# utiasSTARS/pyslam

Hardware: AMD Instinct MI355X
Metric: ms/LM-iter (Jac build + J^T J + Schur solve), stereo BA @ 500k residuals (lower is better)
Workload: dtype f64

## Files before the change

### pyslam_amd/csrc/ps_abi_problem.h

```cpp


const char* ps_last_error(void) { return g_err.c_str(); }

int ps_device_count(void) {
    int n = 0;
    if (hipGetDeviceCount(&n) != hipSuccess) return 0;
    return n;
}

int ps_warm_up(void) {
    static std::once_flag once;
    static int rc = 0;
    std::call_once(once, [] {
        void* p = nullptr;
        if (hipMalloc(&p, 256) != hipSuccess) { rc = fail("hipMalloc failed (no usable HIP device?)"); return; }
        hipLaunchKernelGGL(k_zero4, dim3(1), dim3(256), 0, 0, (size_t)8, (double*)p, (size_t)0, (double*)nullptr, (size_t)0,
                           (double*)nullptr, (size_t)0, (double*)nullptr);
        double hostw[4] = {0, 0, 0, 0};
        (void)hipMemsetAsync(p, 0, 256, 0);
        (void)hipMemcpyAsync((char*)p + 128, p, 64, hipMemcpyDeviceToDevice, 0);
        (void)hipMemcpyAsync(hostw, p, sizeof(hostw), hipMemcpyDeviceToHost, 0);
        if (hipDeviceSynchronize() != hipSuccess) rc = fail("the warm-up launch failed");
        hipFree(p);
        hipFuncAttributes a;
// ... 16 lines not shown
        PS_TOUCH(k_pcg_spmv<6>); PS_TOUCH(k_pcg_spmv<3>); PS_TOUCH(k_ldi_init); PS_TOUCH(k_ldi_update); PS_TOUCH(k_ldi_gemm); PS_TOUCH(k_ldi_mirror);
        PS_TOUCH(k_ldi_ritz); PS_TOUCH(k_ldi_seed_prep); PS_TOUCH(k_ldi_fro_total); PS_TOUCH(k_ldi_pad_identity);
        PS_TOUCH(k_ldi_scaled_dense<6>); PS_TOUCH(k_ldi_sym_unscale<6>); PS_TOUCH(k_ldi_scaled_dense<3>); PS_TOUCH(k_ldi_sym_unscale<3>);
        PS_TOUCH(k_shard_pack<6>); PS_TOUCH(k_shard_unpack<6>); PS_TOUCH(k_publish); PS_TOUCH(k_cov_rhs); PS_TOUCH(k_triangulate<false>);
        PS_TOUCH(k_scale_blocks<3>); PS_TOUCH(k_rows_setup<3, PS_RS_REGS>); PS_TOUCH(k_rows_setup<3, PS_RS_EXACT>); PS_TOUCH(k_coarse_rowsums<3>); PS_TOUCH(k_coarse_matrix<3>);
        PS_TOUCH(k_coarse_chol<3, true>); PS_TOUCH(k_coarse_border<3>); PS_TOUCH(k_coarse_mreduce<3>); PS_TOUCH(k_coarse_xbuild<3>);
        PS_TOUCH(k_coarse_recover<3>); PS_TOUCH(k_cg_fused_lds<3, 8>); PS_TOUCH(k_cg_unscale<3>);
#undef PS_TOUCH
    });
    return rc;
}

int ps_problem_destroy(ps_problem* h) {
    if (!h) return 0;
    if (h->cp_dbg) {
        long long c[8]; hipMemcpy(c, h->cp_dbg, 64, hipMemcpyDeviceToHost);
        int khz = 100000; hipDeviceGetAttribute(&khz, hipDeviceAttributeWallClockRate, 0);
        fprintf(stderr, "k_cg_persist, workgroup 0, %ld launches, us per launch: recurrences %.2f | sync %.2f | products + publish %.2f | gather + sums %.2f "
                "(%.1f failed passes) | dots + sync %.2f | exchanges %lld = %.2f per launch\n", h->cp_launches, c[0] * 1e3 / khz / h->cp_launches,
                c[1] * 1e3 / khz / h->cp_launches, c[2] * 1e3 / khz / h->cp_launches, c[3] * 1e3 / khz / h->cp_launches, (double)c[7] / h->cp_launches,
                c[5] * 1e3 / khz / h->cp_launches, c[6], (double)c[6] / h->cp_launches);
        hipFree(h->cp_dbg);
    }
    if (h->xp_dbg) {
        std::vector<long long> c(3 * 64 * 8); hipMemcpy(c.data(), h->xp_dbg, c.size() * 8, hipMemcpyDeviceToHost);
        int khz = 100000; hipDeviceGetAttribute(&khz, hipDeviceAttributeWallClockRate, 0);
        for (int w = 0; w < 3; ++w) {
            double ph[6] = {0, 0, 0, 0, 0, 0}; int np = 0;
            for (int p = 1; p < 64; ++p) {
                const long long* t = &c[((size_t)w * 64 + p) * 8];
                if (!t[6] || !t[4]) break;
                ph[0] += t[0] - t[6]; ph[1] += t[1] - t[0]; ph[2] += t[2] - t[1]; ph[3] += t[5] - t[2]; ph[4] += t[3] - t[5]; ph[5] += t[4] - t[3]; ++np;
            }
            const double u = 1e3 / khz / std::max(np, 1);
            fprintf(stderr, "k_xcg_persist, workgroup %s, last launch, %d passes, us per pass: t + coarse y %.2f | columns %.2f | products + publish %.2f | "
                    "first gather pass %.2f | rest of the gather %.2f | record sums + dots %.2f | sum %.2f\n", w == 0 ? "0" : (w == 1 ? "nwg/2" : "nwg-1"), np,
// ... 471 lines not shown
```

### pyslam_amd/csrc/ps_abi_solver.h

```cpp

int ps_get_info(ps_problem* h, ps_problem_info* info) {
    if (!h || !info) return fail("null argument");
    info->dof = h->D; info->num_poses = h->P; info->num_reduced = h->nr; info->num_points = h->L;
    info->num_var_points = h->nv; info->num_obs = h->N; info->num_edges = h->F; info->num_priors = 0;
    info->reduced_nnzb = h->nnzb; info->num_pairs = h->npairs;
    info->reduce_count = ((long)h->nnzb + h->nr) / 2 * h->D * h->D + (long)h->nr * h->D + 3;
    info->device_bytes = (int64_t)h->dev_bytes;
    info->cg_restarts = h->cg_fallbacks;
    info->cg_kernel_launches = h->cg_kernel_launches;
    info->ldi_solves = h->ldi_solves; info->ldi_fallbacks = h->ldi_fallbacks; info->ldi_seeds = h->ldi_seeds;
    info->xcg_fused_solves = h->xf_solves; info->xcg_fused_fallbacks = h->xf_fallbacks;
    info->cg_persist_solves = h->cp_launches; info->cg_persist_failures = h->cp_failures;
    info->cg_persist_refused = h->cp_refused; info->persist_cus = h->persist_cus;
    info->persist_cus_needed = h->cp_ok ? h->cp_cus_needed : (h->xp_ok ? h->xp_cus_needed : 0);
    info->landmark_passes_taken_over = h->prelm_used;
    return 0;
}

int ps_eval_cost(ps_problem* h, int include_all_constant, double* cost) {
    if (!h || !cost) return fail("null argument");
    if (include_all_constant && h->fuse_cost == 1 && lm_cost_possible(h)) { if (lm_cost_pass(h, h->lin_lambda, SC_COST)) return -1; }
    else if (cost_pass(h, include_all_constant, SC_COST)) return -1;
    if (read_scalars(h)) return -1;
    *cost = h->h_scalars[SC_COST];
// ... 849 lines not shown
int ps_set_option(ps_problem* h, const char* name, double value) {
    if (!h || !name) return fail("null argument");
    if (!std::strcmp(name, "expect_next")) { h->expect_next = value != 0 && !h->hybrid; return 0; }
    if (!std::strcmp(name, "solve_horizon")) { h->solve_horizon = value < 0 ? -1 : (int)std::min(value, 1e6); return 0; }
    if (!std::strcmp(name, "setup_ride")) {
        h->setup_ride = value != 0 ? 1 : 0;
        h->prelin_valid = h->prelm_valid = false;
        relook_launch_gates(h);
        return 0;
    }
    if (!std::strcmp(name, "rows_regs")) {
        h->rows_regs = value != 0 ? 1 : 0;
        h->prelin_valid = h->prelm_valid = h->ride_valid = false;
        return 0;
    }
    h->prelin_valid = h->prelm_valid = h->ride_valid = false;
    const char* refusal = nullptr;
    const int fx = ps_option_apply(*h, name, value, &refusal);
    if (fx == PS_OPT_UNKNOWN) return fail(std::string("unknown option: ") + name);
    if (fx == PS_OPT_REFUSED) return fail(refusal);
    if (fx & PS_FX_COARSE_REBUILD) h->coarse_built = false;
    if (fx & PS_FX_DROP_FACTOR) h->lci_next = -1;
    if (fx & PS_FX_DROP_SIDE) h->side_todo = false;
    if ((fx & PS_FX_LDI_OFF) && !h->ldi_enable) { h->ldi_cur = -1; if (h->ldi_state != 1) h->ldi_state = 0; }
    if (fx & PS_FX_RELOOK_PATH) relook_path(h);
    relook_launch_gates(h);
    return 0;
}

int ps_get_option(ps_problem* h, const char* name, double* value) {
    if (!h || !name || !value) return fail("null argument");
    const std::string n(name);
    if (n == "lin_zero_list") *value = h->lin_zero_gate ? 1.0 : 0.0;
    else if (n == "lin_fills") *value = (double)h->lin_fills;
    else if (n == "lin_zero_launches") *value = (double)h->lin_zero_launches;
    else if (n == "setup_ride") *value = h->ride_gate ? 1.0 : 0.0;
    else if (n == "factor_launches") *value = (double)h->bjf_launches;
    else if (n == "factors_ridden") *value = (double)h->bjf_ridden;
    else if (n == "factor_plan_mismatches") *value = (double)h->bjf_mismatches;
    else if (n == "rows_regs") *value = (double)h->rows_regs;
    else if (n == "rows_setups") *value = (double)h->rows_setups;
    else if (n == "exact_row_setups") *value = (double)h->exact_row_setups;
    else if (n == "rows_lci_in_lds") *value = h->coarse_built && h->lagx_ok && h->rows_lci_lds ? 1.0 : 0.0;
    else return fail("ps_get_option: no read-back for option: " + n);
    return 0;
}

int ps_reset_solver_state(ps_problem* h) {
    if (!h) return fail("null argument");
    h->prelin_valid = h->prelm_valid = h->ride_valid = false;
    if (!h->solver_touched) {
        static_cast<PsCostHistory&>(*h) = PsCostHistory{};
        return 0;
    }
    h->solver_touched = false;
    HIP_OK(hipStreamSynchronize(h->stream));
    if (h->side) HIP_OK(hipStreamSynchronize(h->side));
    if (h->ldi_stream) HIP_OK(hipStreamSynchronize(h->ldi_stream));
// ... 62 lines not shown
```

### pyslam_amd/csrc/ps_core.hip

```cpp
#include <hip/hip_runtime.h>

#include <algorithm>
#include <array>
#include <map>
#include <atomic>
#include <chrono>
#include <thread>
#include <climits>
#include <cmath>
#include <cstdio>
#include <cstring>
#include <memory>
#include <mutex>
#include <string>
#include <vector>

#include "pyslam_hip.h"
#include "ps_kernels.h"
#include "ps_ransac_core.h"
#include "ps_ransac.h"
#include "ps_k_twoview.h"
#include "ps_k_pnp.h"
#include "ps_k_sim3.h"
#include "ps_photo.h"
// ... 267 lines not shown
    bool xf_one_ok = false, xf_two = false;
    int32_t *xf_cptr = nullptr, *xf_cols = nullptr, *xf_nlo = nullptr, *xf_nhi = nullptr, *xf_rec = nullptr;
    uint16_t* xf_lidx = nullptr;
    double *xf_tq[2] = {}, *xf_ts[2] = {}, *xf_t[2] = {};
    int xf_rmax = 1, xf_nwg = 0, xf_pf = 2;
    size_t xf_nrec = 0;
    long xf_solves = 0, xf_fallbacks = 0;
    bool cp_ok = false;
    bool cp_recovered = false;
    int cp_ntasks = 0, cg_max_launches = 0;
    void* cp_tasks = nullptr;
    int32_t* cp_row_task0 = nullptr;
    unsigned long long* cp_exch = nullptr;
    unsigned cp_salt = 0;
    long cp_launches = 0, cp_failures = 0;
    int persist_dev = 0, persist_cus = 0;
    bool persist_masked = false;
    int cp_cus_needed = 0, xp_cus_needed = 0;
    int persist_held = 0;
    bool params_moved_since_lin = false;
    bool z_foreign = false;
    bool no_repeat = false;
    long cp_refused = 0;
    void persist_release() { if (persist_held) { ps_persist_ledger().release(persist_dev, persist_held); persist_held = 0; } }
    int persist_capacity() const { return persist_masked ? persist_cus / 2 : persist_cus; }
    bool persist_reserve(int need) {
        if (need <= 0 || persist_cus <= 0) return false;
        if (persist_held) return true;
        if (!ps_persist_ledger().reserve(persist_dev, need, persist_capacity())) { ++cp_refused; return false; }
        persist_held = need; return true;
// ... 239 lines not shown
```

### pyslam_amd/csrc/ps_host_cg.h

```cpp

namespace {

struct StageTimer {
    ps_problem* h;
    int stage;
    hipEvent_t a = nullptr, b = nullptr;
    int slot = -1;
    StageTimer(ps_problem* h_, int st, int level = 2) : h(h_), stage(st) {
        if (h->profiling < level) return;
        if (h->profiling == 1 && h->prof_every > 1 &&
            h->prof_tick % h->prof_every != (st == PS_ST_CG_KERNEL ? h->prof_every / 2 : 0)) return;
        if (h->ev_used + 2 > h->ev_pool.size()) {
            for (int i = 0; i < 64; ++i) { hipEvent_t e; hipEventCreate(&e); h->ev_pool.push_back(e); }
        }
        slot = (int)h->ev_used;
        a = h->ev_pool[h->ev_used++];
        b = h->ev_pool[h->ev_used++];
        hipEventRecord(a, h->stream);
    }
    void stop() {
        if (!a) return;
        hipEventRecord(b, h->stream);
        h->pending.push_back({stage, slot});
        a = nullptr;
// ... 311 lines not shown
        h->upload(&h->aug_slot, slot) || h->upload(&h->fine_nnz, fnz)) return -1;
    lap("uploads");
    h->cp_ok = false;
    if (!h->cg_explicit && !split && (long)(nr + ncb) * D <= PS_CP_MAXN) {
        const int rows = nr + ncb;
        std::vector<CpTask> tasks;
        std::vector<int32_t> rt0(rows + 1, 0);
        for (int i = 0; i < rows; ++i) {
            rt0[i] = (int32_t)tasks.size();
            const int w = i < nr ? std::min(arp[i + 1] - arp[i], fnz[i] + ncb) : arp[i + 1] - arp[i];
            const int nt = std::max(1, cdiv(w, PS_CP_TASKB)), per = cdiv(w, nt);
            for (int k = 0; k < nt; ++k) tasks.push_back(CpTask{i, arp[i] + k * per, std::min(arp[i] + w, arp[i] + (k + 1) * per), 0});
        }
        rt0[rows] = (int32_t)tasks.size();
        const int cp_nwg = cdiv((int)tasks.size(), PS_CP_NT / 64);
        int cp_per_cu = 0;
        {
            const void* kfn = D == 6 ? (const void*)k_cg_persist<6> : (const void*)k_cg_persist<3>;
            if (hipOccupancyMaxActiveBlocksPerMultiprocessor(&cp_per_cu, kfn, PS_CP_NT, 0) != hipSuccess) { (void)hipGetLastError(); cp_per_cu = 0; }
        }
        h->cp_cus_needed = cp_per_cu > 0 ? cdiv(cp_nwg, cp_per_cu) : 0;
        if ((long)tasks.size() * D <= (long)PS_CP_MAXEX && h->cp_cus_needed > 0 && h->cp_cus_needed <= h->persist_capacity()) {
            CpTask* dt = nullptr;
            if (h->upload(&dt, tasks) || h->upload(&h->cp_row_task0, rt0) ||
                h->alloc(&h->cp_exch, (size_t)4 * tasks.size() * D)) return -1;
            h->cp_tasks = dt;
            HIP_OK(hipMemsetAsync(h->cp_exch, 0, (size_t)4 * tasks.size() * D * sizeof(unsigned long long), h->stream));
            h->cp_ntasks = (int)tasks.size(); h->cp_salt = 0; h->cp_ok = true;
        }
    }
    if (h->alloc(&h->BSZ, (h->cg_explicit ? eq.size() : (size_t)nr * ncb) * D * D) || h->alloc(&h->Bmat2[0], (size_t)nr * D * D) ||
        h->alloc(&h->bgv, (size_t)nr * D) || h->alloc(&h->SB, (size_t)aci.size() * D * D)) return -1;
    h->Bmat = h->Bmat2[0];
    h->lagx_ok = !h->cg_explicit && !split && h->nc <= 96 && maxlen <= PS_RS_MAXROW;
// ... 371 lines not shown
    return 0;
}

int side_kick(ps_problem* h) {
    if (!h->side_todo) return 0;
    return h->D == 6 ? cg_side_kick<6>(h) : cg_side_kick<3>(h);
}

template <int D>
void cg_fused_launch(ps_problem* h, double tol, int count) {
    const int cap = h->hist_cap;
    const int rows = h->cg_split ? h->nr : h->nr_aug;
    const int ncbs = h->cg_split ? h->ncb : 0;
    const double tol2 = tol * tol;
#ifdef PS_MEASURE
    if (ps_env("PS_CP_CLOCKS") && !h->cp_dbg) { hipMalloc(&h->cp_dbg, 64); hipMemset(h->cp_dbg, 0, 64); }
#endif
    if (h->cg_persist && h->cp_ok && h->G > 0 && h->cg_lds && !h->cg_split && !h->cg_two_level_reduce &&
        !h->cg_ablate && h->cg_launched == 0 && h->cg_max_launches > 0 && h->cg_max_launches <= 4090 && !h->no_repeat &&
        h->persist_reserve(h->cp_cus_needed)) {
        const int nl = h->cg_max_launches;
        if (++h->cp_salt >= (1u << 20)) {
            hipMemsetAsync(h->cp_exch, 0, (size_t)4 * h->cp_ntasks * D * sizeof(unsigned long long), h->stream);
            h->cp_salt = 1;
        }
        hipLaunchKernelGGL((k_cg_persist<D>), dim3(cdiv(h->cp_ntasks, PS_CP_NT / 64)), dim3(PS_CP_NT), 0, h->stream, h->nr_aug * D,
                           h->cp_ntasks, (const CpTask*)h->cp_tasks, h->cp_row_task0, h->acol_idx, h->Saug, h->cg_r[0], h->cg_w[0], h->cg_s[0], h->cg_p,
                           h->cg_xh, h->hist, cap, nl, tol2, h->status, h->scalars, h->cp_exch, h->cp_salt, h->cp_spin, h->cp_dbg,
                           CpRecover{h->nr, h->ncb, h->pnode, h->pw0, h->pw1, h->Linv, h->Lci2[h->lci_cur], h->Bmat, h->x});
        h->cg_launched = nl; h->cg_kernel_launches += 1; ++h->cp_launches;
        h->cp_recovered = true;
        return;
    }
    h->cg_kernel_launches += count;
    for (int i = 0; i < count; ++i, ++h->cg_launched) {
        const int n = h->cg_launched, o = n & 1, nw = o ^ 1;
        const double* tot = h->cg_two_level_reduce ? h->cg_tot : nullptr;
        if (tot && !h->cg_split && n > 0)
            hipLaunchKernelGGL(k_cg_reduce, dim3(1), dim3(1024), 0, h->stream, rows, h->cg_gd[o], h->cg_tot, h->status);
#define PS_CG_LAUNCH(NWV)                                                                                          \
        hipLaunchKernelGGL((k_cg_fused<D, NWV>), dim3(rows), dim3(64 * NWV), 0, h->stream, rows, h->arow_ptr,           \
                           h->acol_idx, h->Saug, h->cg_r[o], h->cg_w[o], h->cg_s[o], h->cg_r[nw], h->cg_w[nw],        \
                           h->cg_s[nw], h->cg_p, h->cg_xh, h->cg_gd[o], h->cg_gd[nw], h->hist, cap, n - 1, tol2,      \
                           h->status, h->scalars, h->nr, h->ell_wf, h->ell_wc, h->cg_ablate, tot, ncbs,              \
                           h->fine_nnz, h->cg_cgd[o], h->cg_U, h->cg_ab)
        if (h->cg_lds && !h->cg_short_rows && !h->cg_split && !tot && !h->cg_ablate && rows <= 1024 &&
// ... 434 lines not shown
```

### pyslam_amd/csrc/ps_k_cg_fused.h

```cpp
#pragma once

template <int D>
__global__ __launch_bounds__(256) void k_block_jacobi_factor(
    int nr, const int32_t* __restrict__ diag_slot, const double* __restrict__ S,
    double* __restrict__ Linv, int32_t* __restrict__ status,
    const double* __restrict__ g, double* __restrict__ r0, double* __restrict__ w0, double* __restrict__ s0,
    double* __restrict__ p0, double* __restrict__ x0,
    const double* __restrict__ poses, const int32_t* __restrict__ pose_of_rid, int basis,
    double* __restrict__ Bmat, double* __restrict__ bg)
{
    constexpr int DD = D * D;
    __shared__ double sc[4][PS_BJF_SCRATCH(D)];
    const int wv = threadIdx.x >> 6, lane = threadIdx.x & 63;
    const int i = blockIdx.x * 4 + wv;
    if (i >= nr) return;
    double a_in = 0.0;
    if (lane < DD) a_in = S[(size_t)diag_slot[i] * DD + lane];
    if (g && lane < D) sc[wv][3 * DD + D + lane] = g[(size_t)i * D + lane];
    const BjFactorOut o{Linv, status, g ? r0 : nullptr, w0, s0, p0, x0, poses, pose_of_rid, basis, Bmat, bg};
    block_jacobi_factor_wave<D>(i, lane, a_in, sc[wv], o);
}

template <int D>
__global__ __launch_bounds__(64) void k_scale_blocks(
// ... 737 lines not shown
    int nr, const int32_t* __restrict__ row_ptr, const int32_t* __restrict__ col_idx, const double* __restrict__ S,
    const double* __restrict__ x, const double* __restrict__ gsaved, double* __restrict__ g)
{
    const int t = blockIdx.x * blockDim.x + threadIdx.x;
    if (t >= nr * D) return;
    const int i = t / D, r = t % D;
    double v = gsaved[t];
    for (int b = row_ptr[i]; b < row_ptr[i + 1]; ++b) {
        const double* sb = S + (size_t)b * D * D + r * D;
        const double* xv = x + (size_t)col_idx[b] * D;
#pragma unroll
        for (int c = 0; c < D; ++c) v -= sb[c] * xv[c];
    }
    g[t] = v;
}
```

### pyslam_amd/csrc/ps_k_cg_persist.h

```cpp
#pragma once

#define PS_CP_NT 512
#define PS_CP_NQ 6
#define PS_CP_TASKB (8 * PS_CP_NQ)
#define PS_CP_NV 4
#define PS_CP_MAXEX (12 * PS_CP_NT)
#define PS_CP_MAXN (PS_CP_NV * PS_CP_NT)
#define PS_CP_LONG 4
#define PS_PERSIST_TIMEOUT_TICKS 100000000LL
#ifndef PS_CP_SLEEP
#define PS_CP_SLEEP 1
#endif

struct CpTask { int32_t row, b0, b1, pad; };
struct CpRecover { int nr, ncb; const int32_t* pnode; const double *pw0, *pw1, *Linv, *Lci, *Bmat; double* x; };

typedef unsigned long long ps_u64;
typedef __attribute__((address_space(1))) ps_u64 ps_gu64;

typedef unsigned ps_u32x4 __attribute__((ext_vector_type(4)));
PS_DEV void cp_put(ps_u64* g, unsigned tag, double v) {
    const ps_u64 b = (ps_u64)__double_as_longlong(v);
    const ps_u32x4 q = {(unsigned)(b & 0xffffffffull), tag, (unsigned)(b >> 32), tag};
    asm volatile("global_store_dwordx4 %0, %1, off sc1\n\ts_nop 1" :: "v"(g), "v"(q) : "memory");
}

PS_DEV ps_u64 cp_get(const ps_u64* buf, unsigned off) {
    return __hip_atomic_load((const ps_gu64*)((const char*)buf + off), __ATOMIC_RELAXED, __HIP_MEMORY_SCOPE_AGENT);
}

template <int D>
__global__ __launch_bounds__(PS_CP_NT) void k_cg_persist(
    int n , int ntasks, const CpTask* __restrict__ tasks,
    const int32_t* __restrict__ row_task0 ,
    const int32_t* __restrict__ acol_idx, const double* __restrict__ Saug,
    const double* __restrict__ r0, const double* __restrict__ w0, const double* __restrict__ s0,
    double* __restrict__ p_io, double* __restrict__ x_io,
    double* __restrict__ hist, int cap, int nlaunch , double tol2,
    int32_t* __restrict__ status, double* __restrict__ scalars,
    ps_u64* __restrict__ exch , unsigned salt, unsigned spin_limit,
    long long* __restrict__ dbg , CpRecover rec)
{
    constexpr int DD = D * D;
    __shared__ double rn[PS_CP_MAXN];
    __shared__ double yc[PS_CP_MAXN];
    __shared__ double red[2][2][PS_CP_NT / 64];
    __shared__ int bad;
    const int t = threadIdx.x, wv = t >> 6, lane = t & 63, kk = lane >> 3, r = lane & 7;
    const int task = blockIdx.x * (PS_CP_NT / 64) + wv;
    const bool chief = blockIdx.x == 0 && t == 0;
    const size_t nex = (size_t)ntasks * D;
    if (t == 0) bad = 0;
    int b0 = 0, b1 = 0;
    if (task < ntasks) { const CpTask tk = tasks[task]; b0 = tk.b0; b1 = tk.b1; }
    int cj[PS_CP_NQ];
    double sv[PS_CP_NQ][D];
#pragma unroll
    for (int q = 0; q < PS_CP_NQ; ++q) {
        const int b = b0 + kk + 8 * q;
        cj[q] = 0;
#pragma unroll
        for (int c = 0; c < D; ++c) sv[q][c] = 0.0;
        if (b < b1 && r < D) {
            cj[q] = acol_idx[b] * D;
            const double* sb = Saug + (size_t)b * DD + r * D;
#pragma unroll
            for (int c = 0; c < D; ++c) sv[q][c] = sb[c];
// ... 2 lines not shown
    double vr[PS_CP_NV], vw[PS_CP_NV], vs[PS_CP_NV], vp[PS_CP_NV], vx[PS_CP_NV];
    int e0[PS_CP_NV], en[PS_CP_NV];
#pragma unroll
    for (int v = 0; v < PS_CP_NV; ++v) {
        const int i = t + v * PS_CP_NT;
        vr[v] = vw[v] = vs[v] = vp[v] = vx[v] = 0.0; e0[v] = 0; en[v] = 0;
        if (i < n) {
            vr[v] = r0[i]; vw[v] = w0[i]; vs[v] = s0[i]; vp[v] = p_io[i]; vx[v] = x_io[i];
            const int row = i / D, ta = row_task0[row];
            e0[v] = ta * D + (i - row * D); en[v] = row_task0[row + 1] - ta;
        }
    }
    int lv = -1, le0 = 0, len = 0;
#pragma unroll
    for (int v = PS_CP_NV - 1; v >= 0; --v) if (en[v] > 2) { lv = v; le0 = e0[v]; len = en[v]; }
    if (status[ST_PCG_DONE]) return;
    double gamma = 0.0, delta = 0.0, inv_gprev = 0.0, inv_aprev = 0.0, thresh = 0.0;
    bool converged = false;
    long long ck[8] = {0, 0, 0, 0, 0, 0, 0, 0};
#define PS_CP_CLK(i) do { if (dbg) { const long long now_ = wall_clock64(); ck[i] += now_ - last_; last_ = now_; } } while (0)
    long long last_ = dbg ? wall_clock64() : 0;
    for (int k = -1; k < nlaunch - 1; ++k) {
        double alpha = 0.0, beta = 0.0;
        if (k >= 0) {
            if (k == 0) thresh = tol2 * gamma;
            if (!(gamma > thresh)) {
                if (chief) { status[ST_PCG_DONE] = (gamma != gamma) ? 2 : 1; scalars[SC_RRFINAL] = gamma; if (k == 0) scalars[SC_RR0] = gamma; }
                converged = !(gamma != gamma);
                break;
            }
            beta = (k == 0) ? 0.0 : gamma * inv_gprev;
            const double denom = (k == 0) ? delta : delta - beta * gamma * inv_aprev;
            alpha = gamma / denom;
            if (!(denom > 0.0)) {
                if (chief) { status[ST_PCG_DONE] = 2; scalars[SC_RRFINAL] = gamma; }
                break;
            }
            if (chief) {
                hist[k] = gamma; hist[cap + k] = alpha; status[ST_PCG_ITERS] = k + 1; scalars[SC_RRFINAL] = gamma;
                if (k == 0) { scalars[SC_THRESH] = thresh; scalars[SC_RR0] = gamma; }
            }
        }
        const double gamma_now = gamma, alpha_now = alpha;
        double gs = 0.0;
#pragma unroll
        for (int v = 0; v < PS_CP_NV; ++v) {
            const int i = t + v * PS_CP_NT;
            const double sn = vw[v] + beta * vs[v];
            const double pn = vr[v] + beta * vp[v];
            const double rnv = cg_rnew(vr[v], vw[v], vs[v], alpha, beta);
            vs[v] = sn; vp[v] = pn; vx[v] += alpha * pn; vr[v] = rnv;
            if (i < n) { rn[i] = rnv; gs += rnv * rnv; }
        }
        double (*rd)[PS_CP_NT / 64] = red[k & 1];
        gs = wave_sum(gs);
        if (lane == 0) rd[0][wv] = gs;
        PS_CP_CLK(0);
        __syncthreads();
        PS_CP_CLK(1);
        double gamma_next = 0.0;
#pragma unroll
        for (int w2 = 0; w2 < PS_CP_NT / 64; ++w2) gamma_next += rd[0][w2];
        if (k >= 0 && k + 1 < nlaunch - 1 && !(gamma_next > thresh)) {
            if (chief) { status[ST_PCG_DONE] = (gamma_next != gamma_next) ? 2 : 1; scalars[SC_RRFINAL] = gamma_next; }
            converged = !(gamma_next != gamma_next);
            break;
        }
        const unsigned tag = salt * 4096u + (unsigned)(k + 2);
        ps_u64* buf = exch + (size_t)(k & 1) * nex * 2;
        {
            double acc = 0.0;
#pragma unroll
            for (int q = 0; q < PS_CP_NQ; ++q) {
                const double* v = rn + cj[q];
#pragma unroll
                for (int c = 0; c < D; ++c) acc += sv[q][c] * v[c];
            }
            acc += __shfl_xor(acc, 8, 64);
            acc += __shfl_xor(acc, 16, 64);
// ... 63 lines not shown
                    if (spins > spin_limit || (long long)wall_clock64() - t_enter > PS_PERSIST_TIMEOUT_TICKS) { bad = 1; break; }
                    if (PS_CP_SLEEP) __builtin_amdgcn_s_sleep(PS_CP_SLEEP);
                    ck[7] += 1;
                }
            }
        }
        PS_CP_CLK(3);
        double ds = 0.0;
#pragma unroll
        for (int v = 0; v < PS_CP_NV; ++v) ds += vw[v] * vr[v];
        ds = wave_sum(ds);
        if (lane == 0) rd[1][wv] = ds;
        __syncthreads();
        PS_CP_CLK(5);
        if (bad) {
            if (t == 0) { status[ST_PCG_DONE] = 2; status[ST_PERSIST_FAIL] = 1; }
            break;
        }
        gamma = gamma_next; delta = 0.0;
#pragma unroll
        for (int w2 = 0; w2 < PS_CP_NT / 64; ++w2) delta += rd[1][w2];
    }
    if (dbg && chief) for (int i = 0; i < 8; ++i) dbg[i] += ck[i];
#undef PS_CP_CLK
    if (blockIdx.x == 0) {
        if (converged && rec.x) {
            const int nc = rec.ncb * D, nf = rec.nr * D;
            __syncthreads();
#pragma unroll
            for (int v = 0; v < PS_CP_NV; ++v) { const int i = t + v * PS_CP_NT; if (i < n) rn[i] = vx[v]; }
            __syncthreads();
            const double* xc = rn + nf;
            for (int base = 0; base < nc; base += PS_CP_NT / 8) {
                const int kq = base + t / 8, sub = t & 7;
                double v = 0.0;
                if (kq < nc) for (int m = kq + sub; m < nc; m += 8) v += rec.Lci[(size_t)m * nc + kq] * xc[m];
                v += __shfl_xor(v, 1, 64); v += __shfl_xor(v, 2, 64); v += __shfl_xor(v, 4, 64);
                if (kq < nc && sub == 0) yc[kq] = v;
            }
            __syncthreads();
            for (int e = t; e < nf; e += PS_CP_NT) {
                const int i = e / D, c = e - i * D, q = rec.pnode[i];
                const double w0 = rec.pw0[i], w1 = rec.pw1[i];
                double z[D];
#pragma unroll
                for (int m = 0; m < D; ++m) z[m] = w0 * yc[q * D + m] + ((q + 1 < rec.ncb) ? w1 * yc[(q + 1) * D + m] : 0.0);
                double v = 0.0;
#pragma unroll
                for (int a = 0; a < D; ++a) {
                    double xhat = rn[i * D + a];
#pragma unroll
                    for (int m = 0; m < D; ++m) xhat += rec.Bmat[(size_t)i * DD + a * D + m] * z[m];
                    v += rec.Linv[(size_t)i * DD + a * D + c] * xhat;
                }
                rec.x[e] = v;
            }
        }
#pragma unroll
        for (int v = 0; v < PS_CP_NV; ++v) {
            const int i = t + v * PS_CP_NT;
            if (i < n) { x_io[i] = vx[v]; p_io[i] = vp[v]; }
        }
    }
}
```

### pyslam_amd/csrc/ps_k_coarse.h

```cpp
#pragma once


PS_DEV double coarse_weight(int j, int q, const int32_t* __restrict__ pnode,
                            const double* __restrict__ pw0, const double* __restrict__ pw1) {
    return (pnode[j] == q) ? pw0[j] : pw1[j];
}

template <int D>
__global__ __launch_bounds__(256) void k_coarse_rowsums(
    int nr, int ncb, const int32_t* __restrict__ run_lo, const int32_t* __restrict__ run_hi,
    const int32_t* __restrict__ acol_idx, const int32_t* __restrict__ pnode,
    const double* __restrict__ pw0, const double* __restrict__ pw1,
    const double* __restrict__ SB ,
    double* __restrict__ SZ, const double* __restrict__ Bmat, double* __restrict__ BSZ )
{
    constexpr int DD = D * D;
    extern __shared__ double srow[];
    const int i = blockIdx.x, nslot = ncb * DD;
    double* sBi = srow + nslot;
    if (threadIdx.x < DD) sBi[threadIdx.x] = Bmat[(size_t)i * DD + threadIdx.x];
    for (int t = threadIdx.x; t < nslot; t += blockDim.x) {
        const int q = t / DD, e = t % DD;
        const int k0 = run_lo[i * ncb + q], k1 = run_hi[i * ncb + q];
        double acc = 0.0;
// ... 587 lines not shown

template <int D>
__global__ __launch_bounds__(256) void k_coarse_recover(
    int nr, int ncb, const int32_t* __restrict__ pnode, const double* __restrict__ pw0,
    const double* __restrict__ pw1, const double* __restrict__ Linv, const double* __restrict__ Lci,
    const double* __restrict__ xh, double* __restrict__ x, const int32_t* __restrict__ gate,
    const double* __restrict__ Bmat)
{
    __shared__ double sy[400];
    if (gate && gate[ST_PCG_DONE] != 1) return;
    const int nc = ncb * D;
    const double* xc = xh + (size_t)nr * D;
    for (int base = 0; base < nc; base += blockDim.x / 8) {
        const int k = base + threadIdx.x / 8, sub = threadIdx.x & 7;
        double v = 0.0;
        if (k < nc) {
#pragma unroll 4
            for (int m = k + sub; m < nc; m += 8) v += Lci[(size_t)m * nc + k] * xc[m];
        }
        v += __shfl_xor(v, 1, 64); v += __shfl_xor(v, 2, 64); v += __shfl_xor(v, 4, 64);
        if (k < nc && sub == 0) sy[k] = v;
    }
    __syncthreads();
    const int t = blockIdx.x * blockDim.x + threadIdx.x;
    if (t >= nr * D) return;
    const int i = t / D, c = t % D, q = pnode[i];
    const double w0 = pw0[i], w1 = pw1[i];
    double z[D];
#pragma unroll
    for (int m = 0; m < D; ++m) z[m] = w0 * sy[q * D + m] + ((q + 1 < ncb) ? w1 * sy[(q + 1) * D + m] : 0.0);
    double v = 0.0;
#pragma unroll
    for (int a = 0; a < D; ++a) {
        double xhat = xh[(size_t)i * D + a];
#pragma unroll
        for (int m = 0; m < D; ++m) xhat += Bmat[(size_t)i * D * D + a * D + m] * z[m];
        v += Linv[(size_t)i * D * D + a * D + c] * xhat;
    }
    x[t] = v;
}

#define PS_RS_THREADS 1024
#define PS_RS_MAXROW 96
#define PS_RS_WAVES 0
#define PS_RS_REGS 1
#define PS_RS_EXACT 2

template <int D, int MODE>
__global__ __launch_bounds__(PS_RS_THREADS) void k_rows_setup(
    int nr, int ncb, const int32_t* __restrict__ row_ptr, const int32_t* __restrict__ col_idx,
    const int32_t* __restrict__ aug_slot, const double* __restrict__ S, const double* __restrict__ Linv,
    const double* __restrict__ Blag, const double* __restrict__ Bcur,
    const int32_t* __restrict__ arow_ptr, const int32_t* __restrict__ fine_nnz,
    const int32_t* __restrict__ run_lo, const int32_t* __restrict__ run_hi,
// ... 232 lines not shown
```

### pyslam_amd/device.py

```python
import ctypes as C

import numpy as np

from pyslam_amd import _native as nat


COVARIANCE_MARGINALS_LIMIT = 12288


def _solve_options(o, opt, linesearch=None):
    o.max_iters, o.allow_nondecreasing_steps = int(opt.max_iters), int(bool(opt.allow_nondecreasing_steps))
    o.max_nondecreasing_steps = int(opt.max_nondecreasing_steps)
    o.linesearch = int(bool(opt.linesearch_max_iters > 0 if linesearch is None else linesearch))
    o.min_update_norm, o.min_cost = float(opt.min_update_norm), float(opt.min_cost)
    o.min_cost_decrease, o.lm_lambda = float(opt.min_cost_decrease), float(getattr(opt, 'lm_lambda', 0.))
    return o


class DeviceProblem:
    def __init__(self, lp, stream=None, extra_pairs=None):
        lib = nat.require_gpu()
        self._lib = lib
        self.lp = lp
        self.dof = lp.dof
# ... 383 lines not shown
    def cg_restarts(self):
        info = nat.ProblemInfo()
        nat.check(self._lib.ps_get_info(self._h, C.byref(info)))
        return int(info.cg_restarts)

    def cg_kernel_launches(self):
        info = nat.ProblemInfo()
        nat.check(self._lib.ps_get_info(self._h, C.byref(info)))
        return int(info.cg_kernel_launches)

    def cg_persist_counts(self):
        info = nat.ProblemInfo()
        nat.check(self._lib.ps_get_info(self._h, C.byref(info)))
        return int(info.cg_persist_solves), int(info.cg_persist_failures)

    def set_option(self, name, value):
        nat.check(self._lib.ps_set_option(self._h, name.encode(), float(value)))

    def get_option(self, name):
        v = C.c_double()
        nat.check(self._lib.ps_get_option(self._h, name.encode(), C.byref(v)))
        return v.value

    def set_profiling(self, level=2):
        nat.check(self._lib.ps_set_profiling(self._h, int(level)))

    def stage_times(self, reset=False):
        ms = (C.c_double * nat.PS_NUM_STAGES)()
        cnt = (C.c_int64 * nat.PS_NUM_STAGES)()
        nat.check(self._lib.ps_get_stage_times(self._h, ms, cnt, int(reset)))
# ... 314 lines not shown
```

Measured before the change: 0.2809.

## Distribute coarse solution recovery across all persistent CG workgroups with LDS prefetch

```diff
diff --git a/pyslam_amd/csrc/ps_abi_problem.h b/pyslam_amd/csrc/ps_abi_problem.h
--- a/pyslam_amd/csrc/ps_abi_problem.h
+++ b/pyslam_amd/csrc/ps_abi_problem.h
@@ -54,12 +54,12 @@
 int ps_problem_destroy(ps_problem* h) {
     if (!h) return 0;
     if (h->cp_dbg) {
-        long long c[8]; hipMemcpy(c, h->cp_dbg, 64, hipMemcpyDeviceToHost);
+        long long c[PS_CP_NCLK]; hipMemcpy(c, h->cp_dbg, sizeof c, hipMemcpyDeviceToHost);
         int khz = 100000; hipDeviceGetAttribute(&khz, hipDeviceAttributeWallClockRate, 0);
         fprintf(stderr, "k_cg_persist, workgroup 0, %ld launches, us per launch: recurrences %.2f | sync %.2f | products + publish %.2f | gather + sums %.2f "
-                "(%.1f failed passes) | dots + sync %.2f | exchanges %lld = %.2f per launch\n", h->cp_launches, c[0] * 1e3 / khz / h->cp_launches,
+                "(%.1f failed passes) | dots + sync %.2f | exchanges %lld = %.2f per launch | prologue %.2f | recovery %.2f\n", h->cp_launches, c[0] * 1e3 / khz / h->cp_launches,
                 c[1] * 1e3 / khz / h->cp_launches, c[2] * 1e3 / khz / h->cp_launches, c[3] * 1e3 / khz / h->cp_launches, (double)c[7] / h->cp_launches,
-                c[5] * 1e3 / khz / h->cp_launches, c[6], (double)c[6] / h->cp_launches);
+                c[5] * 1e3 / khz / h->cp_launches, c[6], (double)c[6] / h->cp_launches, c[8] * 1e3 / khz / h->cp_launches, c[4] * 1e3 / khz / h->cp_launches);
         hipFree(h->cp_dbg);
     }
     if (h->xp_dbg) {
diff --git a/pyslam_amd/csrc/ps_abi_solver.h b/pyslam_amd/csrc/ps_abi_solver.h
--- a/pyslam_amd/csrc/ps_abi_solver.h
+++ b/pyslam_amd/csrc/ps_abi_solver.h
@@ -887,6 +887,17 @@
         h->prelin_valid = h->prelm_valid = h->ride_valid = false;
         return 0;
     }
+    if (!std::strcmp(name, "cg_persist_recover")) {
+        h->cg_persist_recover = value != 0 ? 1 : 0;
+        h->prelin_valid = h->prelm_valid = h->ride_valid = false;
+        return 0;
+    }
+    if (!std::strcmp(name, "cg_persist_recover_lds")) {
+        if (!(value >= 0 && value <= PS_CP_RECOVER_LDS_CAP)) return fail("cg_persist_recover_lds out of range (0 .. 146432 bytes)");
+        h->cg_persist_recover_lds = (int)value;
+        h->prelin_valid = h->prelm_valid = h->ride_valid = false;
+        return 0;
+    }
     h->prelin_valid = h->prelm_valid = h->ride_valid = false;
     const char* refusal = nullptr;
     const int fx = ps_option_apply(*h, name, value, &refusal);
@@ -915,6 +926,11 @@
     else if (n == "rows_setups") *value = (double)h->rows_setups;
     else if (n == "exact_row_setups") *value = (double)h->exact_row_setups;
     else if (n == "rows_lci_in_lds") *value = h->coarse_built && h->lagx_ok && h->rows_lci_lds ? 1.0 : 0.0;
+    else if (n == "cg_persist_recover") *value = (double)h->cg_persist_recover;
+    else if (n == "cg_persist_recover_lds") *value = (double)h->cg_persist_recover_lds;
+    else if (n == "cg_persist_recover_need") *value = h->coarse_built && h->cp_ok ? (double)h->cp_rec_lds : 0.0;
+    else if (n == "cg_persist_recovered") *value = (double)h->cp_rec_inside;
+    else if (n == "cg_persist_recover_fallbacks") *value = (double)h->cp_rec_behind;
     else return fail("ps_get_option: no read-back for option: " + n);
     return 0;
 }
diff --git a/pyslam_amd/csrc/ps_core.hip b/pyslam_amd/csrc/ps_core.hip
--- a/pyslam_amd/csrc/ps_core.hip
+++ b/pyslam_amd/csrc/ps_core.hip
@@ -305,6 +305,11 @@
     unsigned long long* cp_exch = nullptr;
     unsigned cp_salt = 0;
     long cp_launches = 0, cp_failures = 0;
+    int cg_persist_recover = 1;
+    int cg_persist_recover_lds = PS_CP_RECOVER_LDS_CAP;
+    int cp_rec_pp = 0, cp_rec_cols = 0;
+    size_t cp_rec_lds = 0;
+    long cp_rec_inside = 0, cp_rec_behind = 0;
     int persist_dev = 0, persist_cus = 0;
     bool persist_masked = false;
     int cp_cus_needed = 0, xp_cus_needed = 0;
diff --git a/pyslam_amd/csrc/ps_host_cg.h b/pyslam_amd/csrc/ps_host_cg.h
--- a/pyslam_amd/csrc/ps_host_cg.h
+++ b/pyslam_amd/csrc/ps_host_cg.h
@@ -349,10 +349,22 @@
         }
         rt0[rows] = (int32_t)tasks.size();
         const int cp_nwg = cdiv((int)tasks.size(), PS_CP_NT / 64);
+        h->cp_rec_pp = cdiv(nr, cp_nwg); h->cp_rec_cols = 0; h->cp_rec_lds = 0;
+        {
+            bool ascending = true;
+            for (int i = 1; i < nr; ++i) ascending = ascending && pnode[i] >= pnode[i - 1];
+            for (int p0 = 0; p0 < nr && ascending; p0 += h->cp_rec_pp) {
+                const int last = std::min(nr, p0 + h->cp_rec_pp) - 1;
+                h->cp_rec_cols = std::max(h->cp_rec_cols, (std::min(ncb - 1, pnode[last] + 1) - pnode[p0] + 1) * D);
+            }
+            if (ascending && h->cp_rec_pp <= PS_CP_NT) h->cp_rec_lds = cp_recover_lds(D, ncb * D, h->cp_rec_pp, h->cp_rec_cols);
+        }
         int cp_per_cu = 0;
         {
             const void* kfn = D == 6 ? (const void*)k_cg_persist<6> : (const void*)k_cg_persist<3>;
-            if (hipOccupancyMaxActiveBlocksPerMultiprocessor(&cp_per_cu, kfn, PS_CP_NT, 0) != hipSuccess) { (void)hipGetLastError(); cp_per_cu = 0; }
+            const size_t dyn = h->cp_rec_lds <= (size_t)PS_CP_RECOVER_LDS_CAP ? h->cp_rec_lds : 0;
+            if (dyn && ensure_dynamic_lds(kfn, dyn)) return -1;
+            if (hipOccupancyMaxActiveBlocksPerMultiprocessor(&cp_per_cu, kfn, PS_CP_NT, dyn) != hipSuccess) { (void)hipGetLastError(); cp_per_cu = 0; }
         }
         h->cp_cus_needed = cp_per_cu > 0 ? cdiv(cp_nwg, cp_per_cu) : 0;
         if ((long)tasks.size() * D <= (long)PS_CP_MAXEX && h->cp_cus_needed > 0 && h->cp_cus_needed <= h->persist_capacity()) {
@@ -754,7 +766,7 @@
     const int ncbs = h->cg_split ? h->ncb : 0;
     const double tol2 = tol * tol;
 #ifdef PS_MEASURE
-    if (ps_env("PS_CP_CLOCKS") && !h->cp_dbg) { hipMalloc(&h->cp_dbg, 64); hipMemset(h->cp_dbg, 0, 64); }
+    if (ps_env("PS_CP_CLOCKS") && !h->cp_dbg) { hipMalloc(&h->cp_dbg, PS_CP_NCLK * 8); hipMemset(h->cp_dbg, 0, PS_CP_NCLK * 8); }
 #endif
     if (h->cg_persist && h->cp_ok && h->G > 0 && h->cg_lds && !h->cg_split && !h->cg_two_level_reduce &&
         !h->cg_ablate && h->cg_launched == 0 && h->cg_max_launches > 0 && h->cg_max_launches <= 4090 && !h->no_repeat &&
@@ -764,12 +776,15 @@
             hipMemsetAsync(h->cp_exch, 0, (size_t)4 * h->cp_ntasks * D * sizeof(unsigned long long), h->stream);
             h->cp_salt = 1;
         }
-        hipLaunchKernelGGL((k_cg_persist<D>), dim3(cdiv(h->cp_ntasks, PS_CP_NT / 64)), dim3(PS_CP_NT), 0, h->stream, h->nr_aug * D,
+        const bool inside = h->cg_persist_recover && h->cp_rec_lds > 0 && h->cp_rec_lds <= (size_t)h->cg_persist_recover_lds;
+        hipLaunchKernelGGL((k_cg_persist<D>), dim3(cdiv(h->cp_ntasks, PS_CP_NT / 64)), dim3(PS_CP_NT), inside ? h->cp_rec_lds : 0, h->stream, h->nr_aug * D,
                            h->cp_ntasks, (const CpTask*)h->cp_tasks, h->cp_row_task0, h->acol_idx, h->Saug, h->cg_r[0], h->cg_w[0], h->cg_s[0], h->cg_p,
                            h->cg_xh, h->hist, cap, nl, tol2, h->status, h->scalars, h->cp_exch, h->cp_salt, h->cp_spin, h->cp_dbg,
-                           CpRecover{h->nr, h->ncb, h->pnode, h->pw0, h->pw1, h->Linv, h->Lci2[h->lci_cur], h->Bmat, h->x});
+                           CpRecover{h->nr, h->ncb, h->pnode, h->pw0, h->pw1, h->Linv, h->Lci2[h->lci_cur], h->Bmat, inside ? h->x : nullptr,
+                                     h->cp_rec_pp, h->cp_rec_cols});
         h->cg_launched = nl; h->cg_kernel_launches += 1; ++h->cp_launches;
-        h->cp_recovered = true;
+        ++(inside ? h->cp_rec_inside : h->cp_rec_behind);
+        h->cp_recovered = inside;
         return;
     }
     h->cg_kernel_launches += count;
diff --git a/pyslam_amd/csrc/ps_k_cg_fused.h b/pyslam_amd/csrc/ps_k_cg_fused.h
--- a/pyslam_amd/csrc/ps_k_cg_fused.h
+++ b/pyslam_amd/csrc/ps_k_cg_fused.h
@@ -775,3 +775,26 @@
     }
     g[t] = v;
 }
+
+PS_DEV double coarse_recover_ylane(const double* col, int stride, const double* xc, int k, int sub, int nc) {
+    double v = 0.0;
+#pragma unroll 4
+    for (int m = k + sub; m < nc; m += 8) v = fma(col[(size_t)m * stride], xc[m], v);
+    return v;
+}
+template <int D>
+PS_DEV double coarse_recover_entry(const double* y0, const double* y1, double w0, double w1, const double* xh ,
+                                   const double* B , const double* Li , int c) {
+    double z[D];
+#pragma unroll
+    for (int m = 0; m < D; ++m) { const double right = y1 ? w1 * y1[m] : 0.0; z[m] = fma(w0, y0[m], right); }
+    double v = 0.0;
+#pragma unroll
+    for (int a = 0; a < D; ++a) {
+        double xhat = xh[a];
+#pragma unroll
+        for (int m = 0; m < D; ++m) xhat = fma(B[a * D + m], z[m], xhat);
+        v = fma(Li[a * D + c], xhat, v);
+    }
+    return v;
+}
diff --git a/pyslam_amd/csrc/ps_k_cg_persist.h b/pyslam_amd/csrc/ps_k_cg_persist.h
--- a/pyslam_amd/csrc/ps_k_cg_persist.h
+++ b/pyslam_amd/csrc/ps_k_cg_persist.h
@@ -7,13 +7,18 @@
 #define PS_CP_MAXEX (12 * PS_CP_NT)
 #define PS_CP_MAXN (PS_CP_NV * PS_CP_NT)
 #define PS_CP_LONG 4
+#define PS_CP_NCLK 16
 #define PS_PERSIST_TIMEOUT_TICKS 100000000LL
 #ifndef PS_CP_SLEEP
 #define PS_CP_SLEEP 1
 #endif
 
 struct CpTask { int32_t row, b0, b1, pad; };
-struct CpRecover { int nr, ncb; const int32_t* pnode; const double *pw0, *pw1, *Linv, *Lci, *Bmat; double* x; };
+struct CpRecover { int nr, ncb; const int32_t* pnode; const double *pw0, *pw1, *Linv, *Lci, *Bmat; double* x; int pp, maxcols; };
+#define PS_CP_RECOVER_LDS_CAP ((160 - 17) * 1024)
+inline size_t cp_recover_lds(int D, int nc, int pp, int maxcols) {
+    return ((size_t)maxcols * nc + (size_t)pp * (2 * D * D + 2) + maxcols) * sizeof(double) + (size_t)(pp + 2) * sizeof(int32_t);
+}
 
 typedef unsigned long long ps_u64;
 typedef __attribute__((address_space(1))) ps_u64 ps_gu64;
@@ -42,15 +47,50 @@
     long long* __restrict__ dbg , CpRecover rec)
 {
     constexpr int DD = D * D;
-    __shared__ double rn[PS_CP_MAXN];
-    __shared__ double yc[PS_CP_MAXN];
+    __shared__ double rn[PS_CP_MAXN + 2];
     __shared__ double red[2][2][PS_CP_NT / 64];
-    __shared__ int bad;
+    extern __shared__ __attribute__((aligned(16))) double cp_rec[];
+    int& bad = *reinterpret_cast<int*>(&rn[PS_CP_MAXN]);
     const int t = threadIdx.x, wv = t >> 6, lane = t & 63, kk = lane >> 3, r = lane & 7;
     const int task = blockIdx.x * (PS_CP_NT / 64) + wv;
     const bool chief = blockIdx.x == 0 && t == 0;
     const size_t nex = (size_t)ntasks * D;
+    const long long t_entry = dbg ? wall_clock64() : 0;
     if (t == 0) bad = 0;
+    constexpr int PF = 4;
+    const int nc = rec.ncb * D, p0 = blockIdx.x * rec.pp;
+    const int np = rec.x ? max(0, min(rec.nr, p0 + rec.pp) - p0) : 0;
+    int qa = 0, ncols = 0, nlist = 0;
+    if (np > 0) {
+        int32_t* const spn = reinterpret_cast<int32_t*>(cp_rec + rec.maxcols * nc + rec.pp * (2 * DD + 2) + rec.maxcols);
+        qa = rec.pnode[p0];
+        ncols = min((min(rec.ncb - 1, rec.pnode[p0 + np - 1] + 1) - qa + 1) * D, rec.maxcols);
+        nlist = ncols * nc + np * (2 * DD + 2);
+        if (t < np) spn[t] = rec.pnode[p0 + t];
+        if (t == 0) { spn[rec.pp] = qa; spn[rec.pp + 1] = ncols; }
+    }
+    auto rec_src = [&](int idx, int& dst) -> const double* {
+        const int nl = ncols * nc;
+        if (idx < nl) {
+            const int m = idx / ncols, j = idx - m * ncols, k = qa * D + j;
+            dst = j * nc + m;
+            return m >= k ? rec.Lci + (size_t)m * nc + k : nullptr;
+        }
+        const int e = idx - nl, nb = np * DD;
+        dst = rec.maxcols * nc + e;
+        if (e < nb) return rec.Bmat + (size_t)p0 * DD + e;
+        if (e < 2 * nb) return rec.Linv + (size_t)p0 * DD + (e - nb);
+        if (e < 2 * nb + np) return rec.pw0 + p0 + (e - 2 * nb);
+        return rec.pw1 + p0 + (e - 2 * nb - np);
+    };
+    double pfv[PF];
+    int pfd[PF];
+#pragma unroll
+    for (int u = 0; u < PF; ++u) {
+        const int idx = t + u * PS_CP_NT;
+        pfd[u] = -1; pfv[u] = 0.0;
+        if (idx < nlist) { int d = 0; const double* src = rec_src(idx, d); if (src) { pfv[u] = *src; pfd[u] = d; } }
+    }
     int b0 = 0, b1 = 0;
     if (task < ntasks) { const CpTask tk = tasks[task]; b0 = tk.b0; b1 = tk.b1; }
     int cj[PS_CP_NQ];
@@ -83,18 +123,27 @@
     int lv = -1, le0 = 0, len = 0;
 #pragma unroll
     for (int v = PS_CP_NV - 1; v >= 0; --v) if (en[v] > 2) { lv = v; le0 = e0[v]; len = en[v]; }
+#pragma unroll
+    for (int u = 0; u < PF; ++u) if (pfd[u] >= 0) cp_rec[pfd[u]] = pfv[u];
+    for (int base = PF * PS_CP_NT; base < nlist; base += PS_CP_NT) {
+        const int idx = base + t;
+        int d = 0;
+        const double* src = idx < nlist ? rec_src(idx, d) : nullptr;
+        if (src) cp_rec[d] = *src;
+    }
     if (status[ST_PCG_DONE]) return;
     double gamma = 0.0, delta = 0.0, inv_gprev = 0.0, inv_aprev = 0.0, thresh = 0.0;
     bool converged = false;
     long long ck[8] = {0, 0, 0, 0, 0, 0, 0, 0};
 #define PS_CP_CLK(i) do { if (dbg) { const long long now_ = wall_clock64(); ck[i] += now_ - last_; last_ = now_; } } while (0)
     long long last_ = dbg ? wall_clock64() : 0;
+    if (dbg && chief) dbg[8] += last_ - t_entry;
     for (int k = -1; k < nlaunch - 1; ++k) {
         double alpha = 0.0, beta = 0.0;
         if (k >= 0) {
             if (k == 0) thresh = tol2 * gamma;
             if (!(gamma > thresh)) {
-                if (chief) { status[ST_PCG_DONE] = (gamma != gamma) ? 2 : 1; scalars[SC_RRFINAL] = gamma; if (k == 0) scalars[SC_RR0] = gamma; }
+                if (chief) { atomicMax(&status[ST_PCG_DONE], (gamma != gamma) ? 2 : 1); scalars[SC_RRFINAL] = gamma; if (k == 0) scalars[SC_RR0] = gamma; }
                 converged = !(gamma != gamma);
                 break;
             }
@@ -102,7 +151,7 @@
             const double denom = (k == 0) ? delta : delta - beta * gamma * inv_aprev;
             alpha = gamma / denom;
             if (!(denom > 0.0)) {
-                if (chief) { status[ST_PCG_DONE] = 2; scalars[SC_RRFINAL] = gamma; }
+                if (chief) { atomicMax(&status[ST_PCG_DONE], 2); scalars[SC_RRFINAL] = gamma; }
                 break;
             }
             if (chief) {
@@ -131,7 +180,7 @@
 #pragma unroll
         for (int w2 = 0; w2 < PS_CP_NT / 64; ++w2) gamma_next += rd[0][w2];
         if (k >= 0 && k + 1 < nlaunch - 1 && !(gamma_next > thresh)) {
-            if (chief) { status[ST_PCG_DONE] = (gamma_next != gamma_next) ? 2 : 1; scalars[SC_RRFINAL] = gamma_next; }
+            if (chief) { atomicMax(&status[ST_PCG_DONE], (gamma_next != gamma_next) ? 2 : 1); scalars[SC_RRFINAL] = gamma_next; }
             converged = !(gamma_next != gamma_next);
             break;
         }
@@ -225,46 +274,50 @@
         __syncthreads();
         PS_CP_CLK(5);
         if (bad) {
-            if (t == 0) { status[ST_PCG_DONE] = 2; status[ST_PERSIST_FAIL] = 1; }
+            if (t == 0) { atomicMax(&status[ST_PCG_DONE], 2); status[ST_PERSIST_FAIL] = 1; }
             break;
         }
         gamma = gamma_next; delta = 0.0;
 #pragma unroll
         for (int w2 = 0; w2 < PS_CP_NT / 64; ++w2) delta += rd[1][w2];
     }
-    if (dbg && chief) for (int i = 0; i < 8; ++i) dbg[i] += ck[i];
 #undef PS_CP_CLK
+    const long long t_left = dbg ? wall_clock64() : 0;
+    if (converged && rec.x) {
+        __syncthreads();
+#pragma unroll
+        for (int v = 0; v < PS_CP_NV; ++v) { const int i = t + v * PS_CP_NT; if (i < n) rn[i] = vx[v]; }
+        __syncthreads();
+        const int nc = rec.ncb * D, p0 = blockIdx.x * rec.pp, np = max(0, min(rec.nr, p0 + rec.pp) - p0);
+        if (np > 0) {
+            const double* sLc = cp_rec;
+            const double* sOp = sLc + rec.maxcols * nc;
+            double* sy = cp_rec + rec.maxcols * nc + rec.pp * (2 * DD + 2);
+            const int32_t* spn = reinterpret_cast<const int32_t*>(sy + rec.maxcols);
+            const int qa = spn[rec.pp], ncols = spn[rec.pp + 1];
+            const double* xc = rn + rec.nr * D;
+            for (int base = 0; base < ncols; base += PS_CP_NT / 8) {
+                const int j = base + t / 8, sub = t & 7;
+                double v = 0.0;
+                if (j < ncols) v = coarse_recover_ylane(sLc + j * nc, 1, xc, qa * D + j, sub, nc);
+                v += __shfl_xor(v, 1, 64); v += __shfl_xor(v, 2, 64); v += __shfl_xor(v, 4, 64);
+                if (j < ncols && sub == 0) sy[j] = v;
+            }
+            __syncthreads();
+            const double *sB = sOp, *sLi = sOp + np * DD, *sw0 = sOp + 2 * np * DD, *sw1 = sw0 + np;
+            for (int e = t; e < np * D; e += PS_CP_NT) {
+                const int il = e / D, c = e - il * D, q = spn[il];
+                rec.x[(size_t)p0 * D + e] = coarse_recover_entry<D>(sy + (q - qa) * D, (q + 1 < rec.ncb) ? sy + (q + 1 - qa) * D : nullptr,
+                                                                    sw0[il], sw1[il], rn + (p0 + il) * D, sB + il * DD, sLi + il * DD, c);
+            }
+        }
+    }
     if (blockIdx.x == 0) {
-        if (converged && rec.x) {
-            const int nc = rec.ncb * D, nf = rec.nr * D;
+        if (dbg) {
             __syncthreads();
-#pragma unroll
-            for (int v = 0; v < PS_CP_NV; ++v) { const int i = t + v * PS_CP_NT; if (i < n) rn[i] = vx[v]; }
-            __syncthreads();
-            const double* xc = rn + nf;
-            for (int base = 0; base < nc; base += PS_CP_NT / 8) {
-                const int kq = base + t / 8, sub = t & 7;
-                double v = 0.0;
-                if (kq < nc) for (int m = kq + sub; m < nc; m += 8) v += rec.Lci[(size_t)m * nc + kq] * xc[m];
-                v += __shfl_xor(v, 1, 64); v += __shfl_xor(v, 2, 64); v += __shfl_xor(v, 4, 64);
-                if (kq < nc && sub == 0) yc[kq] = v;
-            }
-            __syncthreads();
-            for (int e = t; e < nf; e += PS_CP_NT) {
-                const int i = e / D, c = e - i * D, q = rec.pnode[i];
-                const double w0 = rec.pw0[i], w1 = rec.pw1[i];
-                double z[D];
-#pragma unroll
-                for (int m = 0; m < D; ++m) z[m] = w0 * yc[q * D + m] + ((q + 1 < rec.ncb) ? w1 * yc[(q + 1) * D + m] : 0.0);
-                double v = 0.0;
-#pragma unroll
-                for (int a = 0; a < D; ++a) {
-                    double xhat = rn[i * D + a];
-#pragma unroll
-                    for (int m = 0; m < D; ++m) xhat += rec.Bmat[(size_t)i * DD + a * D + m] * z[m];
-                    v += rec.Linv[(size_t)i * DD + a * D + c] * xhat;
-                }
-                rec.x[e] = v;
+            if (t == 0) {
+                ck[4] = wall_clock64() - t_left;
+                for (int i = 0; i < 8; ++i) dbg[i] += ck[i];
             }
         }
 #pragma unroll
diff --git a/pyslam_amd/csrc/ps_k_coarse.h b/pyslam_amd/csrc/ps_k_coarse.h
--- a/pyslam_amd/csrc/ps_k_coarse.h
+++ b/pyslam_amd/csrc/ps_k_coarse.h
@@ -625,10 +625,7 @@
     for (int base = 0; base < nc; base += blockDim.x / 8) {
         const int k = base + threadIdx.x / 8, sub = threadIdx.x & 7;
         double v = 0.0;
-        if (k < nc) {
-#pragma unroll 4
-            for (int m = k + sub; m < nc; m += 8) v += Lci[(size_t)m * nc + k] * xc[m];
-        }
+        if (k < nc) v = coarse_recover_ylane(Lci + k, nc, xc, k, sub, nc);
         v += __shfl_xor(v, 1, 64); v += __shfl_xor(v, 2, 64); v += __shfl_xor(v, 4, 64);
         if (k < nc && sub == 0) sy[k] = v;
     }
@@ -636,19 +633,8 @@
     const int t = blockIdx.x * blockDim.x + threadIdx.x;
     if (t >= nr * D) return;
     const int i = t / D, c = t % D, q = pnode[i];
-    const double w0 = pw0[i], w1 = pw1[i];
-    double z[D];
-#pragma unroll
-    for (int m = 0; m < D; ++m) z[m] = w0 * sy[q * D + m] + ((q + 1 < ncb) ? w1 * sy[(q + 1) * D + m] : 0.0);
-    double v = 0.0;
-#pragma unroll
-    for (int a = 0; a < D; ++a) {
-        double xhat = xh[(size_t)i * D + a];
-#pragma unroll
-        for (int m = 0; m < D; ++m) xhat += Bmat[(size_t)i * D * D + a * D + m] * z[m];
-        v += Linv[(size_t)i * D * D + a * D + c] * xhat;
-    }
-    x[t] = v;
+    x[t] = coarse_recover_entry<D>(sy + q * D, (q + 1 < ncb) ? sy + (q + 1) * D : nullptr, pw0[i], pw1[i], xh + (size_t)i * D,
+                                   Bmat + (size_t)i * D * D, Linv + (size_t)i * D * D, c);
 }
 
 #define PS_RS_THREADS 1024
diff --git a/pyslam_amd/device.py b/pyslam_amd/device.py
--- a/pyslam_amd/device.py
+++ b/pyslam_amd/device.py
@@ -421,6 +421,9 @@
         nat.check(self._lib.ps_get_info(self._h, C.byref(info)))
         return int(info.cg_persist_solves), int(info.cg_persist_failures)
 
+    def cg_persist_recover_counts(self):
+        return int(self.get_option('cg_persist_recovered')), int(self.get_option('cg_persist_recover_fallbacks'))
+
     def set_option(self, name, value):
         nat.check(self._lib.ps_set_option(self._h, name.encode(), float(value)))
 
```

Result: faster. 0.2757 (median of 6 runs) (-1.8%).
